# vpc-ccg/haslr

Hardware: AMD Instinct MI355X
Metric: long-read bases/sec through backbone+consensus; GFA match + FASTA %identity (higher is better)
Workload: dtype int32

## Files before the change

### haslr_amd/csrc/kernels/poa.hip

```cpp
#include <type_traits>

#include "kernels.h"

namespace hxk {

namespace {

#include "poa_graph.inl"
#include "poa_dp.inl"
#include "poa_edge.inl"
#include "poa_update.inl"

#define PHASE(k) do { if (tid == 0) { long long _n = clock64(); ph[k] += (unsigned long long)(_n - tc); tc = _n; } } while (0)
#if POA_PHASE_FLAVOUR == POA_PHASE_GUSTAGES
#define GU_T0() do { __syncthreads(); if (tid == 0) tg = clock64(); } while (0)
#define GU_T(k) do { __syncthreads(); if (tid == 0) { long long _n = clock64(); ph[k] += (unsigned long long)(_n - tg); tg = _n; } } while (0)
#else
#define GU_T0() do { } while (0)
#define GU_T(k) do { } while (0)
#endif
#if POA_PHASE_FLAVOUR == POA_PHASE_DPSUB
#define SUBT(k) do { if (tid == 0) { long long _n = clock64(); ph[k] += (unsigned long long)(_n - tc2); tc2 = _n; } } while (0)
#define SUBT0() do { if (tid == 0) tc2 = clock64(); } while (0)
#else
#define SUBT(k) do { } while (0)
#define SUBT0() do { } while (0)
#endif
#define HX_DP_DISPATCH(Lq, Vq, nsq, Tq) do { \
        if (((Lq) + 1 + GM * NP * DL - 1) / (GM * NP * DL) <= (uint32_t)CM) {     \
            dp_rows<CM, DIR, PRUNE, MAXNT == 64>(g, H, Dm, Dw, W, WH, seq, Lq, Vq, ring, R, ring_w, match, mismatch, gap, wmail.box, wmail.consumed, sink_row, sink_score, SINK_LDS, nsq, cl, ph + PW_BUILD0, Tq, (prune_pct >> 16) & 1u, ph + PW_PRUNE0, ED.hrows); \
        } else sOk = ES_INTERNAL; } while (0)

template <int MAXNT, int CM, bool DIR, bool PRUNE>
__device__ __forceinline__ void poa_edge(const uint32_t eidx, const uint32_t mem, const PoaSlot SL, const PoaEdge* __restrict__ edges,
                                         const PoaSeq* __restrict__ seqs, const uint8_t* __restrict__ packed, const uint64_t* __restrict__ read_off,
                                         const uint32_t* __restrict__ read_len, const PoaPools& P, int32_t match, int32_t mismatch, int32_t gap,
                                         char* cns, uint32_t* cns_len, uint32_t* status, unsigned long long* cells, unsigned long long* phase,
                                         uint32_t poll_limit, uint32_t lds_bytes, uint32_t max_indeg, uint32_t dp_lanes, uint32_t prune_pct) {
    __shared__ unsigned long long ph[POA_PHASE_WORDS];
    __shared__ long long tc;
    if (threadIdx.x == 0) { for (int k = 0; k < POA_PHASE_WORDS; k++) ph[k] = 0; tc = clock64(); ph[PW_BEGIN] = pw_pack(pw_lo(wall_clock64(), PW_SPLIT_CLOCK), (unsigned long long)((__builtin_amdgcn_s_getreg(63492) & 0x7fffu) | ((__builtin_amdgcn_s_getreg(63508) & 15u) << 15)), PW_SPLIT_CLOCK); }
#if POA_PHASE_FLAVOUR == POA_PHASE_GUSTAGES
    long long tg = 0;
#endif
#if POA_PHASE_FLAVOUR == POA_PHASE_DPSUB
    __shared__ long long tc2;
#endif
    const PoaEdge ED = edges[eidx];
    const uint32_t tid = threadIdx.x, NT = blockDim.x;
    const uint32_t DL = dp_lanes ? dp_lanes : NT;
    extern __shared__ int32_t ring[];
    G g;
    bind_graph(g, P, SL, ED);
    int32_t* H = P.H + SL.h_off;
    uint8_t* Dm = DIR ? P.dir + SL.d_off : nullptr;
    uint8_t* Dw = DIR ? P.dirw + SL.w_off : nullptr;
    const uint32_t GM = ED.members;
    const uint32_t ring_w = CM * (DL >> 6) * 65u;
    uint32_t R = 0;
    {
        const uint32_t fit = lds_bytes / (ring_w * 4u);
        R = fit >= 8 ? 8 : fit >= 4 ? 4 : fit >= 2 ? 2 : 0;
        if (fit < 1) R = 0xffffffffu;
    }
    uint8_t* seq = P.seq + SL.seq_off;
    const uint32_t W = (ED.lmax + 1 + 31) & ~31u;
    const uint32_t NP = GM == 1 && ED.passes > 1 ? ED.passes : 1u;
    const uint32_t WT = GM * NP * (DL >> 6);
    const uint32_t WH = W + (WT > 1 ? (WT + 3u) & ~3u : 0u);

    constexpr uint32_t SINK_LDS = MAXNT <= 256 ? 128 : MAXNT < 1024 ? 256 : SINK_CAP;
    __shared__ WaveMailT<MAXNT / 64> wmail;
    __shared__ uint32_t lds_u[16];
    __shared__ uint32_t sV, sE, sNaln, sOk, sNsink, sNcand, sBestKey, sWalkN, sWalkI, sWalkJ;
    __shared__ int sBestI;
    __shared__ uint32_t sink_row[SINK_LDS];
    __shared__ int sink_score[SINK_LDS];
    __shared__ uint32_t sCtl;
    __shared__ unsigned long long sCells;
    __shared__ int sPrevScore, sNewT; __shared__ uint32_t sPrevLen, sRetry;
    if (tid == 0) { sV = 0; sE = 0; sOk = R != 0xffffffffu ? ES_OK : ES_INTERNAL; sCells = 0; sPrevScore = 0; sPrevLen = 0; sRetry = 0; sNewT = PRUNE_OFF; }
    if constexpr (MAXNT > 64) {
        for (uint32_t q = tid; q < (MAXNT / 64 - 1) * WAVE_MBOX; q += NT) wmail.box[q] = 0ull;
        if (tid < MAXNT / 64) wmail.consumed[tid] = 0u;
    }
    __syncthreads();
    uint32_t* csy = P.csync + (uint64_t)eidx * CW_STRIDE;
    int32_t* sinkbuf = P.sinkbuf + (uint64_t)eidx * (1 + 2 * SINK_CAP);
    DpCl cl;
    cl.mem = mem; cl.members = GM; cl.stride = ED.vcap + 1; cl.tag0 = 0;
    cl.mbox = P.mbox + (NP > 1 ? SL.mbox_off : ED.cl_off); cl.err = csy + CW_ERR; cl.poll_limit = poll_limit; cl.lanes = DL;
    const uint32_t topo_lcap = lds_bytes >= 24 * 1024 ? 1024u : lds_bytes >= 8 * 1024 ? 256u : 128u;
    const uint32_t topo_lines = lds_bytes >= 24 * 1024 ? 64u : lds_bytes >= 8 * 1024 ? 16u : 8u;
    const uint32_t topo_fixed = topo_lcap * 4 + topo_lines * 256 + topo_lines * 4;
    uint32_t* t_stack = reinterpret_cast<uint32_t*>(ring);
    uint4* t_cache = reinterpret_cast<uint4*>(reinterpret_cast<uint8_t*>(ring) + topo_lcap * 4);
    uint32_t* t_tags = reinterpret_cast<uint32_t*>(reinterpret_cast<uint8_t*>(ring) + topo_lcap * 4 + topo_lines * 256);
    uint8_t* st_lds = reinterpret_cast<uint8_t*>(ring) + topo_fixed;
    uint32_t* tmp_u32 = reinterpret_cast<uint32_t*>(g.pred);
    auto exact_order = [&](uint32_t Vn, uint32_t* out) {
        const bool wave_dfs = topo_fixed + 16 <= lds_bytes;
        const bool st_in_lds = wave_dfs && (uint64_t)Vn + topo_fixed + 16 <= lds_bytes;
        uint8_t* st = st_in_lds ? st_lds : g.mark;
        if (wave_dfs) { for (uint32_t i = tid; i < Vn; i += NT) st[i] = 4u; }
        else { for (uint32_t i = tid; i < Vn; i += NT) { g.mark[i] = 0; g.check[i] = 1; } }
        __threadfence_block();
        __syncthreads();
        if (wave_dfs) {
            uint32_t* ranks = reinterpret_cast<uint32_t*>(g.score);
#if POA_PHASE_FLAVOUR == POA_PHASE_DPSUB
            long long tq0 = clock64();
#endif
            if (tid < 64) toposort_rank(g, Vn, st, t_stack, t_cache, t_tags, ranks, topo_lcap, topo_lines);
#if POA_PHASE_FLAVOUR == POA_PHASE_DPSUB
            if (tid == 0) ph[PW_P2_TOPO] += (unsigned long long)(clock64() - tq0);
#endif
            __threadfence_block();
            __syncthreads();
            for (uint32_t i = tid; i < Vn; i += NT) tmp_u32[i] = g.rank2node[ranks[i]];
            __syncthreads();
            if (out != tmp_u32) { for (uint32_t i = tid; i < Vn; i += NT) out[i] = tmp_u32[i]; }
        } else if (tid == 0) toposort(g, Vn, out);
        __syncthreads();
    };

    uint32_t att = 0;
    for (uint32_t k = ED.seq_begin; mem > 0 || k < ED.seq_end; k += (mem == 0 ? 1u : 0u)) {
        uint32_t L, V;
        if (mem == 0 && sOk != ES_OK) break;
        if (mem == 0) {
            const PoaSeq q = seqs[k];
            L = q.len;
            {
                const uint8_t* rp = packed + read_off[q.rid];
                const uint32_t rlen = read_len[q.rid];
                for (uint32_t j = tid; j < L; j += NT) {
                    uint32_t p = q.strand == 0 ? q.spos + j : rlen - 1 - (q.spos + j);
                    uint8_t b = (rp[p >> 2] >> ((p & 3) * 2)) & 3;
                    seq[j] = q.strand == 0 ? b : (uint8_t)(3 - b);
                }
            }
            __syncthreads();
            PHASE(PW_DECODE);
            V = sV;
            SUBT0();
        } else {
            if (tid == 0) {
                uint32_t v = 0;
                for (uint32_t spin = 0;; spin++) {
                    v = ld_dev(csy + CW_GO);
                    if (v == CL_ABORT || v >= att + 1) break;
                    if (spin > poll_limit) { st_dev(csy + CW_ERR, 1u); v = CL_ABORT; break; }
                    __builtin_amdgcn_s_sleep(32);
                }
                sCtl = v;
            }
            __syncthreads();
            if (sCtl == CL_ABORT) break;
            __builtin_amdgcn_fence(__ATOMIC_ACQUIRE, "agent");
            V = ld_dev(csy + CW_V); L = ld_dev(csy + CW_L);
        }
        if (mem == 0) SUBT(PW_P2_PUBLISH);
        int thrT = PRUNE_OFF;
        if constexpr (PRUNE) {
            if (mem == 0 && (prune_pct & 0xffffu) != 0u && sPrevLen != 0u && V < (1u << 20)) {
                const float f = (float)(prune_pct & 0xffffu) * 0.01f;
                float e = (float)sPrevScore * (float)L / (float)sPrevLen;
                e = e >= 0.f ? e * f : e * (2.f - f);
                thrT = (int)fmaxf((float)PRUNE_OFF, floorf(e));
            }
        }
    redo_dp:
        att++;
        if (GM > 1) {
            if (mem == 0) cluster_publish(csy, V, L, thrT, att);
            else if constexpr (PRUNE) thrT = (int)ld_dev(csy + CW_THRESHOLD);
        }
        if (V > 0) {
            uint32_t ns = 0xffffffffu;
#if POA_PHASE_FLAVOUR == POA_PHASE_MEMBERS
            const long long td0 = clock64();
            if (tid == 0) ph[PW_P3_WAIT] = 0;
#endif
            if (NP > 1) {
                for (uint32_t pass = 0; pass < NP && (uint64_t)pass * DL * CM <= L; pass++) {
                    cl.mem = pass; cl.members = NP;
                    HX_DP_DISPATCH(L, V, ns, thrT);
                    __threadfence();
                    __syncthreads();
                }
                cl.mem = 0; cl.members = 1;
            } else
            HX_DP_DISPATCH(L, V, ns, thrT);
#if POA_PHASE_FLAVOUR == POA_PHASE_MEMBERS
            if (tid == 0 && phase) atomicAdd(&phase[(uint64_t)eidx * POA_PHASE_WORDS + PW_P3_MEMBER0 + min(mem, (uint32_t)(PW_N_BUILD - 1))], pw_pack(0, ph[PW_P3_WAIT] >> 10, PW_SPLIT_HALF) | pw_pack((unsigned long long)(clock64() - td0) >> 10, 0, PW_SPLIT_HALF));
#endif
            if (ns != 0xffffffffu) sNsink = ns;
            cl.tag0 += V;
        }
        if (mem > 0) {
            __syncthreads();
            if (V > 0 && L / (DL * (uint32_t)CM) == mem) {
                const uint32_t nsk = min(sNsink, SINK_LDS);
                if (tid == 0) sinkbuf[0] = (int32_t)sNsink;
                for (uint32_t q = tid; q < nsk; q += NT) { sinkbuf[1 + q] = (int32_t)sink_row[q]; sinkbuf[1 + SINK_CAP + q] = sink_score[q]; }
            }
            __threadfence();
            __syncthreads();
            if (tid == 0) __hip_atomic_fetch_add(csy + CW_DONE, 1u, __ATOMIC_RELAXED, __HIP_MEMORY_SCOPE_AGENT);
            continue;
        }
        SUBT(PW_P2_OWN);
        if (V > 0) {
            if (GM > 1) {
                cluster_wait_members(csy, GM, att, poll_limit);
                __builtin_amdgcn_fence(__ATOMIC_ACQUIRE, "agent");
                if (L / (DL * (uint32_t)CM) != 0) {
                    const uint32_t nsk_all = (uint32_t)sinkbuf[0], nsk = min(nsk_all, SINK_LDS);
                    for (uint32_t q = tid; q < nsk; q += NT) { sink_row[q] = (uint32_t)sinkbuf[1 + q]; sink_score[q] = sinkbuf[1 + SINK_CAP + q]; }
                    if (tid == 0) sNsink = nsk_all;
                }
            }
            __syncthreads();
            if (tid == 0 && ld_dev(csy + CW_ERR) && sOk == ES_OK) sOk = ld_dev(csy + CW_ERR) == 2u ? ES_INTERNAL : ES_STALLED;
            __syncthreads();
            if (sOk != ES_OK) break;
            SUBT(PW_P2_WAIT);
            if (tid == 0) {
                if (sNsink > SINK_LDS) sOk = ES_SINKS;
                int best = INT32_MIN + 1024; uint32_t ncand = 0, first = 0;
                const uint32_t nsk = min(sNsink, SINK_LDS);
                for (uint32_t q = 0; q < nsk; q++) if (sink_score[q] > best) best = sink_score[q];
                for (uint32_t q = 0; q < nsk; q++) if (sink_score[q] == best) { if (!ncand) first = q; sink_row[ncand++] = sink_row[q]; }
                (void)first;
                if constexpr (PRUNE) {
                    sRetry = thrT > PRUNE_OFF && sOk == ES_OK && best < thrT;
                    if (sRetry) { sNewT = nsk ? max(best, PRUNE_OFF) : PRUNE_OFF; ph[PW_PRUNE_REPEATED]++; }
                    else { sPrevScore = best; sPrevLen = L; ph[PW_PRUNE_THRESHOLDS] += thrT > PRUNE_OFF; }
                }
                sNcand = ncand; sBestI = ncand ? (int)sink_row[0] : -1; sBestKey = 0xffffffffu;
                lds_u[WALK_AT_I] = 0; lds_u[WALK_AT_J] = 0; lds_u[WALK_DONE] = 0;
                if (ncand > 1 && ncand <= 8 && lds_bytes >= 640u && !(PRUNE && sRetry)) {
                    constexpr uint32_t UCAP = 32, SCAP = 256;
                    uint32_t* U = reinterpret_cast<uint32_t*>(ring);
                    uint8_t* mk = reinterpret_cast<uint8_t*>(U + UCAP);
                    uint8_t* ck = mk + UCAP;
                    uint8_t* stk = ck + UCAP;
                    uint32_t nu = 0, cn[8];
                    bool ok = true;
                    auto find = [&](uint32_t x) -> uint32_t { for (uint32_t q = 0; q < nu; q++) if (U[q] == x) return q; return NONE; };
                    auto addcol = [&](uint32_t x) {
                        if (find(x) != NONE) return;
                        const uint32_t na = g.n_aligned[x];
                        if (nu + 1 + na > UCAP) { ok = false; return; }
                        U[nu++] = x;
                        for (uint32_t k = 0; k < na; k++) U[nu++] = g.aligned[3 * x + k];
                    };
                    for (uint32_t c = 0; c < ncand; c++) { cn[c] = g.rank2node[sink_row[c] - 1]; if (ok) addcol(cn[c]); }
                    for (uint32_t q = 0; q < nu && ok; q++)
                        for (uint32_t e = g.out_head[U[q]]; e != NONE && ok; e = g.e_next_out[e]) addcol(g.e_to[e]);
                    if (ok) {
                        for (uint32_t q = 1; q < nu; q++) {
                            const uint32_t x = U[q]; uint32_t r = q;
                            while (r > 0 && U[r - 1] > x) { U[r] = U[r - 1]; r--; }
                            U[r] = x;
                        }
                        for (uint32_t q = 0; q < nu; q++) { mk[q] = 0; ck[q] = 1; }
                        auto cand_of = [&](uint32_t x) -> uint32_t { for (uint32_t c = 0; c < ncand; c++) if (cn[c] == x) return c; return NONE; };
                        uint32_t win = NONE;
                        for (uint32_t root = 0; root < nu && win == NONE && ok; root++) {
                            if (mk[root]) continue;
                            uint32_t sp = 0;
                            stk[sp++] = (uint8_t)root;
                            while (sp && win == NONE && ok) {
                                const uint32_t q = stk[sp - 1], n = U[q];
                                bool valid = true;
                                if (mk[q] != 2) {
                                    for (uint32_t e = g.in_head[n]; e != NONE; e = g.e_next_in[e]) {
                                        const uint32_t f = find(g.e_from[e]);
                                        if (f != NONE && mk[f] != 2) { if (sp < SCAP) stk[sp++] = (uint8_t)f; else ok = false; valid = false; }
                                    }
                                    const uint32_t na = g.n_aligned[n];
                                    if (ck[q])
                                        for (uint32_t k = 0; k < na; k++) {
                                            const uint32_t a = find(g.aligned[3 * n + k]);
                                            if (mk[a] != 2) { if (sp < SCAP) stk[sp++] = (uint8_t)a; else ok = false; ck[a] = 0; valid = false; }
                                        }
                                    if (valid) {
                                        mk[q] = 2;
                                        if (ck[q]) {
                                            win = cand_of(n);
                                            for (uint32_t k = 0; k < na && win == NONE; k++) win = cand_of(g.aligned[3 * n + k]);
                                        }
                                    } else mk[q] = 1;
                                }
                                if (valid) sp--;
                            }
                        }
                        if (ok && win != NONE) { sBestI = (int)sink_row[win]; sNcand = 1; }
                    }
                }
            }
            __syncthreads();
            if constexpr (PRUNE) {
                if (sRetry) {
                    thrT = sNewT;
                    __syncthreads();
                    if (tid == 0) sRetry = 0;
                    goto redo_dp;
                }
            }
            if (sNcand > 1 && sOk == ES_OK) {
                if (tid == 0) ph[PW_P2_TIES] += 1;
                exact_order(V, tmp_u32);
                const uint32_t nc = sNcand;
                for (uint32_t r = tid; r < V; r += NT) {
                    const uint32_t n = tmp_u32[r];
                    for (uint32_t q = 0; q < nc; q++)
                        if (g.rank2node[sink_row[q] - 1] == n) atomicMin(&sBestKey, (r << 10) | q);
                }
                __syncthreads();
                if (tid == 0) { sBestI = (int)sink_row[sBestKey & 1023u]; atomicAdd(&ph[PW_ORDER], 0ull); }
            }
            __syncthreads();
            SUBT(PW_P2_END);
            PHASE(PW_DP);
            if (DIR) {
                if (tid < 64) {
                    const uint32_t ln = tid;
                    if (ln == 0) sCells += (unsigned long long)V * L;
                    uint32_t i = (uint32_t)__builtin_amdgcn_readfirstlane(sBestI), j = L, na = 0;
                    int pn = 0, pp = 0;
                    uint32_t nwalk = 0, iend = 0, jend = 0;
                    bool tail = false;
                    while (!(i == 0 && j == 0)) {
                        if (__builtin_expect(na > V + L + 2u, 0)) { if (ln == 0) sOk = ES_INTERNAL; break; }
                        if (i == 0) {
                            if (na & 63u) { const uint32_t base = na & ~63u; if (ln < na - base) { g.aln_node[base + ln] = pn; g.aln_pos[base + ln] = pp; } }
                            tail = true;
                            nwalk = na; iend = 0; jend = j;
                            for (uint32_t q = ln; q < j; q += 64) { g.aln_node[na + q] = -1; g.aln_pos[na + q] = (int32_t)(j - 1 - q); }
                            na += j; j = 0;
                            break;
                        }
                        const uint32_t ti = i, ct = j | 1u;
                        if (NT > 64 && ln == 0) { st_wg(&lds_u[WALK_AT_I], ti); st_wg(&lds_u[WALK_AT_J], ct); }
                        const int32_t bs = ((int32_t)ct - 31) >> 1;
                        uint32_t w0 = 0, w1 = 0, w2 = 0, w3 = 0, mt = 0, pv0 = 0, pv1 = 0, qo = 0, qw = 0;
                        if (ti > ln) {
                            const uint8_t* rowp = Dm + (uint64_t)(ti - ln) * (W >> 1) + bs;
                            __builtin_memcpy(&w0, rowp, 4); __builtin_memcpy(&w1, rowp + 4, 4); __builtin_memcpy(&w2, rowp + 8, 4); __builtin_memcpy(&w3, rowp + 12, 4);
                            const uint32_t rr = ti - 1 - ln;
                            mt = g.row_meta[rr]; qo = g.row_pred_off[rr]; if (mt & 32u) qw = g.wslot[rr];
                            pv0 = (mt >> META_NP) == 0 ? 0u : (g.row_pred0[rr] & 0x0fffffffu) + 1;
                            pv1 = (g.row_pred1[rr] & 0x0fffffffu) + 1;
                        }
                        uint32_t ilo = ti > 63u ? ti - 63u : 1u;
                        asm volatile("" : "+s"(ilo));
                        const int32_t jb0 = 2 * bs;
                        const unsigned long long wmask = __ballot((mt & 32u) != 0);
                        if (mt & 32u) { w0 = 0x88888888u; w1 = 0x88888888u; w2 = 0x88888888u; w3 = 0x88888888u; }
                        for (;;) {
                            const uint32_t dr = ti - i, jb = (uint32_t)((int32_t)j - jb0);
                            const uint32_t wsa = (uint32_t)__builtin_amdgcn_readlane((int)w0, (int)dr), wsb = (uint32_t)__builtin_amdgcn_readlane((int)w1, (int)dr);
                            const uint32_t wsc = (uint32_t)__builtin_amdgcn_readlane((int)w2, (int)dr), wsd = (uint32_t)__builtin_amdgcn_readlane((int)w3, (int)dr);
                            const uint32_t wsh = ((jb & 16u) ? ((jb & 8u) ? wsd : wsc) : ((jb & 8u) ? wsb : wsa)) >> (4 * (jb & 7u));
                            const uint32_t n4 = wsh & 15u;
                            const uint32_t pva = (uint32_t)__builtin_amdgcn_readlane((int)pv0, (int)dr), pvb = (uint32_t)__builtin_amdgcn_readlane((int)pv1, (int)dr);
                            uint32_t ni, nj;
                            asm("s_andn2_b32 %0, 3, %2\n\ts_cselect_b32 %0, %4, %3\n\ts_bitcmp1_b32 %2, 3\n\ts_cselect_b32 %0, %0, %5\n\t"
                                "s_and_b32 %1, %2, 12\n\ts_cmp_lg_u32 %1, 8\n\ts_subb_u32 %1, %6, 0"
                                : "=&s"(ni), "=&s"(nj) : "s"(wsh), "s"(pva), "s"(pvb), "s"(i), "s"(j) : "scc");
                            if (__builtin_expect((n4 & 10u) == 8u, 0)) {
                                uint32_t type = n4 >> 2, slot = 3u - (n4 & 3u), later = 1u, pv = slot == 0 ? pva : pvb;
                                if ((uint32_t)(wmask >> dr) & 1u) {
                                    const uint32_t d = (uint32_t)__builtin_amdgcn_readfirstlane((int)Dw[(uint64_t)__builtin_amdgcn_readlane((int)qw, (int)dr) * W + j]);
                                    type = d >> 4; slot = 15u - (d & 15u); later = slot >= 2 && type > 1u;
                                    pv = slot == 0 ? pva : pvb;
                                }
                                if (later != 0)
                                    pv = ((uint32_t)__builtin_amdgcn_readfirstlane((int)g.pred_rank[(uint32_t)__builtin_amdgcn_readlane((int)qo, (int)dr) + slot]) & 0x0fffffffu) + 1;
                                ni = type > 1u ? pv : i;
                                nj = j - (uint32_t)(type != 2u);
                            }
                            {
                                const int el = (int)(na & 63u);
                                int m0_keep;
                                asm volatile("s_mov_b32 %2, m0\n\ts_mov_b32 m0, %3\n\ts_nop 0\n\tv_writelane_b32 %0, %4, m0\n\tv_writelane_b32 %1, %5, m0\n\ts_mov_b32 m0, %2"
                                             : "+v"(pn), "+v"(pp), "=&s"(m0_keep) : "s"(el), "s"(i), "s"(j));
                            }
                            if (__builtin_expect((na & 63u) == 63u, 0)) {
                                asm volatile("" ::: "memory");
                                g.aln_node[na - 63 + ln] = pn; g.aln_pos[na - 63 + ln] = pp;
                            }
                            na++;
                            i = ni; j = nj;
                            if ((int32_t)((i - ilo) | (uint32_t)((int32_t)j - jb0)) < 0) break;
                        }
                    }
                    if (!tail) {
                        if (na & 63u) { const uint32_t base = na & ~63u; if (ln < na - base) { g.aln_node[base + ln] = pn; g.aln_pos[base + ln] = pp; } }
                        nwalk = na; iend = 0; jend = 0;
                    }
                    if (ln == 0) { sNaln = na; lds_u[WALK_N] = nwalk; lds_u[WALK_I] = iend; lds_u[WALK_J] = jend; st_wg(&lds_u[WALK_DONE], 1u); }
                } else if (tid < 128) {
                    const uint32_t hl = tid - 64u;
                    uint32_t last_i = 0xffffffffu, sink = 0;
                    for (uint32_t spin = 0; spin < (1u << 26); spin++) {
                        if (ld_wg(&lds_u[WALK_DONE])) break;
                        const uint32_t pi_ = ld_wg(&lds_u[WALK_AT_I]), pc = ld_wg(&lds_u[WALK_AT_J]);
                        if (pi_ == last_i) { __builtin_amdgcn_s_sleep(8); continue; }
                        last_i = pi_;
                        for (uint32_t hk = 0; hk < 2; hk++) {
                        const uint32_t d = 64u + hl + 64u * hk;
                        if (pi_ > d) {
                            const uint32_t r = pi_ - d, rr = r - 1;
                            const uint8_t* rowp = Dm + (uint64_t)r * (W >> 1);
                            const uint32_t c_lo = pc > d ? pc - d : 0u, c_hi = pc > d / 3u ? pc - d / 3u : 0u;
                            uint32_t a0, a1;
                            __builtin_memcpy(&a0, rowp + ((c_lo >> 1) & ~3u), 4); __builtin_memcpy(&a1, rowp + ((c_hi >> 1) & ~3u), 4);
                            const uint32_t mt = g.row_meta[rr], qo = g.row_pred_off[rr];
                            sink ^= a0 ^ a1 ^ g.row_pred0[rr] ^ g.row_pred1[rr];
                            if ((mt >> META_NP) > 2u) sink ^= g.pred_rank[qo + 2] ^ g.pred_rank[qo + (mt >> META_NP) - 1];
                            if (mt & 32u) { const uint8_t* wp = Dw + (uint64_t)g.wslot[rr] * W; sink ^= wp[c_lo] ^ wp[(c_lo + c_hi) >> 1] ^ wp[c_hi]; }
                        }
                        }
                    }
                    asm volatile("" :: "v"(sink));
                }
                __syncthreads();
                if (tid == 0) { sWalkN = lds_u[WALK_N]; sWalkI = lds_u[WALK_I]; sWalkJ = lds_u[WALK_J]; }
                __syncthreads();
            } else if (tid == 0) {
                sCells += (unsigned long long)V * L;
                uint32_t i = (uint32_t)sBestI, j = L, na = 0;
                while (!DIR && !(i == 0 && j == 0)) {
                    const int hij = H[(uint64_t)i * WH + j];
                    uint32_t pi_ = i, pj_ = j;
                    bool found = false;
                    uint32_t po = 0, pe = 0;
                    if (i != 0) { po = g.row_pred_off[i - 1]; pe = g.row_pred_off[i]; }
                    if (i != 0 && j != 0) {
                        const int mc = seq[j - 1] == (uint8_t)(g.row_meta[i - 1] & 3u) ? match : mismatch;
                        if (po == pe) { if (hij == H[j - 1] + mc) { pi_ = 0; pj_ = j - 1; found = true; } }
                        else for (uint32_t p = po; p < pe && !found; p++) {
                            uint32_t pr = (g.pred_rank[p] & 0x0fffffffu) + 1;
                            if (hij == H[(uint64_t)pr * WH + j - 1] + mc) { pi_ = pr; pj_ = j - 1; found = true; }
                        }
                    }
                    if (!found && i != 0) {
                        if (po == pe) { if (hij == H[j] + gap) { pi_ = 0; pj_ = j; found = true; } }
                        else for (uint32_t p = po; p < pe && !found; p++) {
                            uint32_t pr = (g.pred_rank[p] & 0x0fffffffu) + 1;
                            if (hij == H[(uint64_t)pr * WH + j] + gap) { pi_ = pr; pj_ = j; found = true; }
                        }
                    }
                    if (!found) { pi_ = i; pj_ = j - 1; }
                    g.aln_node[na] = i == pi_ ? -1 : (int32_t)g.rank2node[i - 1];
                    g.aln_pos[na] = j == pj_ ? -1 : (int32_t)(j - 1);
                    na++;
                    i = pi_; j = pj_;
                }
                sNaln = na; sWalkN = 0;
            }
        } else {
            if (tid == 0) { sNaln = 0; sWalkN = 0; }
            if (GM > 1) cluster_wait_members(csy, GM, att, poll_limit);
        }
        __syncthreads();
        if (sOk != ES_OK) break;
        PHASE(PW_TRACEBACK);
        const uint32_t V_old = sV;
        graph_update(g, seq, L, sNaln, sWalkN, sWalkI, sWalkJ, lds_u, &sV, &sE, &sNcand, &sOk);
        PHASE(PW_GRAPH);
        __syncthreads();
        if (sOk != ES_OK) break;
        order_update(g, V_old, sV, L, lds_u);
        PHASE(PW_ORDER);
        __syncthreads();
        csr_rebuild<MAXNT, DIR>(g, sV, R, max_indeg, ED.hrows, ED.wrows, lds_u, &sOk, ph, phase != nullptr, eidx, k == ED.seq_begin, k + 1 == ED.seq_end);
        __syncthreads();
        PHASE(PW_CSR);
    }
    if (mem > 0) return;
    if (GM > 1 && tid == 0) st_dev(csy + CW_GO, CL_ABORT);
    long long t_cns = 0;
    if (tid == 0) t_cns = clock64();
    if (sOk == ES_OK && sV) {
        if (tid < 64) { const uint32_t cl_ = consensus_fast_wave(g, sV, cns + ED.cns_off); if (tid == 0) sCtl = cl_; }
        __syncthreads();
        if (sCtl == NONE) {
            if (tid == 0) ph[PW_REFCNS] = 1;
            exact_order(sV, g.rank2node);
            for (uint32_t r = tid; r < sV; r += NT) g.node2rank[g.rank2node[r]] = r;
            __syncthreads();
            csr_rebuild<MAXNT, DIR>(g, sV, R, 0xffffffffu, 0xffffffffu, 0xffffffffu, lds_u, &sOk, ph, false, eidx, false, false);
            __threadfence_block();
            __syncthreads();
            if (tid < 64) { const uint32_t cl_ = consensus_wave(g, sV, cns + ED.cns_off); if (tid == 0) sCtl = cl_; }
            __syncthreads();
        }
    }
    if (tid == 0) {
        if (sOk == ES_INTERNAL) { status[eidx] = HXE_SPOS_RANGE << 8; cns_len[eidx] = 0; }
        else if (sOk == ES_OVERFLOW) { status[eidx] = HXE_POA_OVERFLOW; cns_len[eidx] = 0; }
        else if (sOk == ES_NODIR) { status[eidx] = HXE_POA_NODIR; cns_len[eidx] = 0; }
        else if (sOk == ES_FARROWS) { status[eidx] = HXE_POA_FARROWS; cns_len[eidx] = 0; }
        else if (sOk == ES_SINKS) { status[eidx] = HXE_POA_SINKS; cns_len[eidx] = 0; }
        else if (sOk == ES_WIDEROWS) { status[eidx] = HXE_POA_WIDEROWS; cns_len[eidx] = 0; }
        else if (sOk == ES_STALLED) { status[eidx] = HXE_POA_STALLED; cns_len[eidx] = 0; }
        else {
            status[eidx] = 0; cns_len[eidx] = !sV ? 0 : sCtl; atomicAdd(cells, sCells);
#if POA_PHASE_FLAVOUR == POA_PHASE_ROWSTATS
            if (phase) atomicAdd(&ph[PW_SEQS_NODES], pw_pack(0, sV, PW_SPLIT_HALF));
#endif
        }
        ph[PW_CNS] = (unsigned long long)(clock64() - t_cns);
        PHASE(PW_GRAPH);
        ph[PW_END] = pw_lo(wall_clock64(), PW_SPLIT_CLOCK);
#if POA_PHASE_FLAVOUR == POA_PHASE_MEMBERS
        if (phase) for (int k = 0; k < PW_N_PHASES; k++) phase[(uint64_t)eidx * POA_PHASE_WORDS + k] = ph[k];
#else
        if (phase) for (int k = 0; k < POA_PHASE_WORDS; k++) phase[(uint64_t)eidx * POA_PHASE_WORDS + k] = ph[k];
#endif
    }
}
#undef HX_DP_DISPATCH
#undef SUBT0
#undef SUBT
#undef GU_T
#undef GU_T0
#undef PHASE

template <int MAXNT, int CM, bool DIR, bool PERSIST, bool PRUNE>
__global__ void __launch_bounds__(MAXNT, (CM == 8 && DIR ? 4 : 1)) k_poa(const PoaEdge* __restrict__ edges, const uint32_t* __restrict__ order, uint32_t n_items,
                                            const PoaSlot* __restrict__ slots, uint32_t* __restrict__ counter ,
                                            const uint32_t* __restrict__ btab , const PoaSeq* __restrict__ seqs, const uint8_t* __restrict__ packed, const uint64_t* __restrict__ read_off,
                                            const uint32_t* __restrict__ read_len, PoaPools P, int32_t match, int32_t mismatch, int32_t gap,
                                            char* cns, uint32_t* cns_len, uint32_t* status, unsigned long long* cells, unsigned long long* phase,
                                            uint32_t poll_limit, uint32_t lds_bytes, uint32_t max_indeg, uint32_t dp_lanes, uint32_t prune_pct,
                                            uint32_t* __restrict__ started ) {
    __shared__ uint32_t sNext;
    if (started && threadIdx.x == 0) __hip_atomic_fetch_add(started, 1u, __ATOMIC_RELAXED, __HIP_MEMORY_SCOPE_SYSTEM);
    uint32_t kb = 0, nbk = 0;
    bool own_first = false;
    if (PERSIST) { nbk = btab[0] & 0xffffu; own_first = (btab[0] >> 16) & 1u; while (kb + 1 < nbk && blockIdx.x >= btab[1 + kb]) kb++; }
    for (uint32_t round = 0;; round++) {
        uint32_t eidx, mem = 0;
        PoaSlot SL;
        if (!PERSIST) {
            eidx = order[blockIdx.x] & 0x00ffffffu; mem = order[blockIdx.x] >> 24;
            if (eidx == 0x00ffffffu) return;
            SL = slots[edges[eidx].slot];
        } else {
            if (round) __syncthreads();
            if (threadIdx.x == 0) {
                const uint32_t* ib = btab + 1 + nbk;
                const uint32_t* est = ib + nbk + 1;
                uint32_t idx = 0xffffffffu;
                for (uint32_t tries = 0; tries < 64 && idx == 0xffffffffu; tries++) {
                    uint32_t best = 0xffffffffu, bv = 0;
                    for (uint32_t k = kb; k < nbk; k++) {
                        const uint32_t b0 = ib[k], b1 = ib[k + 1], cur = __hip_atomic_load(counter + k, __ATOMIC_RELAXED, __HIP_MEMORY_SCOPE_AGENT);
                        if (cur >= b1 - b0) continue;
                        const uint32_t v = est[b0 + cur];
                        if (best == 0xffffffffu || v > bv) { best = k; bv = v; }
                        if (own_first && k == kb) break;
                    }
                    if (best == 0xffffffffu) break;
                    const uint32_t t = ib[best] + atomicAdd(counter + best, 1u);
                    if (t < ib[best + 1]) idx = t;
                }
                sNext = idx;
            }
            __syncthreads();
            const uint32_t idx = sNext;
            if (idx == 0xffffffffu) return;
            eidx = order[idx] & 0x00ffffffu;
            SL = slots[blockIdx.x];
        }
        poa_edge<MAXNT, CM, DIR, PRUNE>(eidx, mem, SL, edges, seqs, packed, read_off, read_len, P, match, mismatch, gap, cns, cns_len, status, cells, phase, poll_limit, lds_bytes, max_indeg, dp_lanes, prune_pct);
        if (!PERSIST) return;
    }
}

}

#if !defined(HX_POA_PART) || HX_POA_PART == 64
#define HX_POA_HAS_64 1
#endif
#if !defined(HX_POA_PART) || HX_POA_PART == 256
#define HX_POA_HAS_256 1
#endif
#if !defined(HX_POA_PART) || HX_POA_PART == 512
#define HX_POA_HAS_512 1
#endif
#if !defined(HX_POA_PART) || HX_POA_PART == 1024
#define HX_POA_HAS_1024 1
#endif
#define HX_LAUNCH(MNT, CMV, DIRV, PERS, PRN) do { \
        (void)hipFuncSetAttribute((const void*)k_poa<MNT, CMV, DIRV, PERS, PRN>, hipFuncAttributeMaxDynamicSharedMemorySize, 142 * 1024); \
        if (q.occupancy) { (void)hipOccupancyMaxActiveBlocksPerMultiprocessor(q.occupancy, (const void*)k_poa<MNT, CMV, DIRV, PERS, PRN>, q.block_threads, q.ring_bytes); break; } \
        k_poa<MNT, CMV, DIRV, PERS, PRN><<<q.n_blocks, q.block_threads, q.ring_bytes, s>>>(q.edges, q.order, q.n_items, q.slots, q.counter, q.btab, q.seqs, q.packed, q.read_off, q.read_len, q.pools, q.match, q.mismatch, q.gap, \
                                                                       q.cns, q.cns_len, q.status, q.cells, q.phase, q.poll_limit, q.ring_bytes, q.max_indeg, q.dp_lanes, q.prune_pct, q.started); } while (0)
#define HX_LAUNCH_CM(MNT, CMV) do { if (q.use_dir && q.counter) HX_LAUNCH(MNT, CMV, true, true, false); else if (q.use_dir) HX_LAUNCH(MNT, CMV, true, false, false); else HX_LAUNCH(MNT, CMV, false, false, false); } while (0)
#define HX_LAUNCH_PR(MNT, CMV) do { if (q.counter) HX_LAUNCH(MNT, CMV, true, true, true); else HX_LAUNCH(MNT, CMV, true, false, true); } while (0)
#define HX_POA_RUN_PART(MNT, LAST_CM) \
    void poa_run_##MNT(const PoaLaunch& q, hipStream_t s, bool prune) { \
        const int cm = q.cm; \
        if constexpr (MNT == 256 || MNT == 1024) { if (prune && cm <= 2 && !q.counter) { HX_LAUNCH(MNT, 2, true, false, true); return; } } \
        if (prune) { if (cm <= 4) HX_LAUNCH_PR(MNT, 4); else HX_LAUNCH_PR(MNT, 8); return; } \
        if constexpr (MNT == 256 || MNT == 1024) { if (cm <= 2 && q.use_dir && !q.counter) { HX_LAUNCH(MNT, 2, true, false, false); return; } }    \
        if (cm <= 4) HX_LAUNCH_CM(MNT, 4); else if (cm <= 8) HX_LAUNCH_CM(MNT, 8); else if (cm <= 16 || LAST_CM == 16) HX_LAUNCH_CM(MNT, 16); else HX_LAUNCH_CM(MNT, LAST_CM); \
    }
#ifdef HX_POA_HAS_64
HX_POA_RUN_PART(64, 32)
#endif
#ifdef HX_POA_HAS_256
HX_POA_RUN_PART(256, 32)
#endif
#ifdef HX_POA_HAS_512
HX_POA_RUN_PART(512, 16)
#endif
#ifdef HX_POA_HAS_1024
HX_POA_RUN_PART(1024, 32)
#endif
#undef HX_POA_RUN_PART
#undef HX_LAUNCH_CM
#undef HX_LAUNCH_PR
#undef HX_LAUNCH

#if !defined(HX_POA_PART) || HX_POA_PART == 64
void poa_run_64(const PoaLaunch&, hipStream_t, bool);
void poa_run_256(const PoaLaunch&, hipStream_t, bool);
void poa_run_512(const PoaLaunch&, hipStream_t, bool);
void poa_run_1024(const PoaLaunch&, hipStream_t, bool);
void poa_run(const PoaLaunch& q, hipStream_t s) {
    if (!q.n_blocks || !q.n_items) return;
    if (q.counter && !q.use_dir) return;
    const bool prune = poa_prune_ok(q.use_dir, q.cm) && q.prune_pct != 0u;
    const int mnt = poa_kernel_lanes(q.block_threads);
    if (mnt == 64) poa_run_64(q, s, prune);
    else if (mnt == 256) poa_run_256(q, s, prune);
    else if (mnt == 512) poa_run_512(q, s, prune);
    else poa_run_1024(q, s, prune);
}
#endif

}
```

Measured before the change: 2.256 billion.

## Precompute per-lane traceback step table and walk with scalar asm state machine

```diff
diff --git a/haslr_amd/csrc/kernels/poa.hip b/haslr_amd/csrc/kernels/poa.hip
--- a/haslr_amd/csrc/kernels/poa.hip
+++ b/haslr_amd/csrc/kernels/poa.hip
@@ -30,6 +30,33 @@
         if (((Lq) + 1 + GM * NP * DL - 1) / (GM * NP * DL) <= (uint32_t)CM) {     \
             dp_rows<CM, DIR, PRUNE, MAXNT == 64>(g, H, Dm, Dw, W, WH, seq, Lq, Vq, ring, R, ring_w, match, mismatch, gap, wmail.box, wmail.consumed, sink_row, sink_score, SINK_LDS, nsq, cl, ph + PW_BUILD0, Tq, (prune_pct >> 16) & 1u, ph + PW_PRUNE0, ED.hrows); \
         } else sOk = ES_INTERNAL; } while (0)
+
+#define HX_WS(C, T, OFF, RA, RB) \
+    "Ls" #C "_%=:\n\tv_readlane_b32 %[x], %[" T "], %[" RA "]\n\ts_bfe_u32 %[" RB "], %[x], " #OFF "|0x80000\n\ts_cmp_lt_u32 %[" RB "], 64\n\ts_cbranch_scc0 Lx" #C "_%=\n\t" \
+    "s_or_b32 %[w], %[" RA "], (" #C "+2)<<6\n\tv_writelane_b32 %[rec], %[w], m0\n\ts_add_u32 m0, m0, 1\n"
+#define HX_WX(C, RA, RB) \
+    "Lx" #C "_%=:\n\ts_bitcmp1_b32 %[" RB "], 7\n\ts_cbranch_scc1 Ld" #C "_%=\n\ts_cmp_lt_u32 m0, 32\n\ts_cbranch_scc0 Ld" #C "_%=\n\t" \
+    "s_or_b32 %[w], %[" RA "], (" #C "+2)<<6\n\tv_writelane_b32 %[rec], %[w], m0\n\ts_add_u32 m0, m0, 1\n\ts_and_b32 %[" RA "], %[" RB "], 63\n\ts_branch Ls" #C "_%=\n" \
+    "Ld" #C "_%=:\n\ts_mov_b32 %[x], %[" RB "]\n\ts_mov_b32 %[dr], %[" RA "]\n\ts_movk_i32 %[c], " #C "\n\ts_branch Lend_%=\n"
+#define HX_WE(C) "Le" #C "_%=:\n\ts_mov_b32 %[drb], %[dr]\n\ts_branch Ls" #C "_%=\n"
+#define HX_WPAIR(CO, CE, TO, TE, OFF) HX_WS(CO, TO, OFF, "dr", "drb") HX_WS(CE, TE, OFF, "drb", "dr")
+#define HX_WXPAIR(CO, CE) HX_WX(CO, "dr", "drb") HX_WX(CE, "drb", "dr") HX_WE(CE)
+#define HX_WGO(C, L) "s_cmp_eq_u32 %[c], " #C "\n\ts_cbranch_scc1 " L #C "_%=\n\t"
+#define HX_WALK_ASM \
+    "s_mov_b32 %[keep], m0\n\ts_mov_b32 m0, %[el]\n\ts_nop 0\n\t" \
+    "s_cmp_lt_u32 %[c], 8\n\ts_cbranch_scc1 Lg0_%=\n\ts_cmp_lt_u32 %[c], 16\n\ts_cbranch_scc1 Lg1_%=\n\ts_cmp_lt_u32 %[c], 24\n\ts_cbranch_scc1 Lg2_%=\n\t" \
+    HX_WGO(31, "Ls") HX_WGO(30, "Le") HX_WGO(29, "Ls") HX_WGO(28, "Le") HX_WGO(27, "Ls") HX_WGO(26, "Le") HX_WGO(25, "Ls") "s_branch Le24_%=\n" \
+    "Lg2_%=:\n\t" HX_WGO(23, "Ls") HX_WGO(22, "Le") HX_WGO(21, "Ls") HX_WGO(20, "Le") HX_WGO(19, "Ls") HX_WGO(18, "Le") HX_WGO(17, "Ls") "s_branch Le16_%=\n" \
+    "Lg1_%=:\n\t" HX_WGO(15, "Ls") HX_WGO(14, "Le") HX_WGO(13, "Ls") HX_WGO(12, "Le") HX_WGO(11, "Ls") HX_WGO(10, "Le") HX_WGO(9, "Ls") "s_branch Le8_%=\n" \
+    "Lg0_%=:\n\t" HX_WGO(7, "Ls") HX_WGO(6, "Le") HX_WGO(5, "Ls") HX_WGO(4, "Le") HX_WGO(3, "Ls") HX_WGO(2, "Le") HX_WGO(1, "Ls") "s_branch Le0_%=\n" \
+    HX_WPAIR(31, 30, "t7", "t6", 24) HX_WPAIR(29, 28, "t7", "t6", 16) HX_WPAIR(27, 26, "t7", "t6", 8) HX_WPAIR(25, 24, "t7", "t6", 0) \
+    HX_WPAIR(23, 22, "t5", "t4", 24) HX_WPAIR(21, 20, "t5", "t4", 16) HX_WPAIR(19, 18, "t5", "t4", 8) HX_WPAIR(17, 16, "t5", "t4", 0) \
+    HX_WPAIR(15, 14, "t3", "t2", 24) HX_WPAIR(13, 12, "t3", "t2", 16) HX_WPAIR(11, 10, "t3", "t2", 8) HX_WPAIR(9, 8, "t3", "t2", 0) \
+    HX_WPAIR(7, 6, "t1", "t0", 24) HX_WPAIR(5, 4, "t1", "t0", 16) HX_WPAIR(3, 2, "t1", "t0", 8) HX_WPAIR(1, 0, "t1", "t0", 0) \
+    "\ts_mov_b32 %[x], 0\n\ts_branch Lend_%=\n" \
+    HX_WXPAIR(31, 30) HX_WXPAIR(29, 28) HX_WXPAIR(27, 26) HX_WXPAIR(25, 24) HX_WXPAIR(23, 22) HX_WXPAIR(21, 20) HX_WXPAIR(19, 18) HX_WXPAIR(17, 16) \
+    HX_WXPAIR(15, 14) HX_WXPAIR(13, 12) HX_WXPAIR(11, 10) HX_WXPAIR(9, 8) HX_WXPAIR(7, 6) HX_WXPAIR(5, 4) HX_WXPAIR(3, 2) HX_WXPAIR(1, 0) \
+    "Lend_%=:\n\ts_mov_b32 %[el], m0\n\ts_mov_b32 m0, %[keep]"
 
 template <int MAXNT, int CM, bool DIR, bool PRUNE>
 __device__ __forceinline__ void poa_edge(const uint32_t eidx, const uint32_t mem, const PoaSlot SL, const PoaEdge* __restrict__ edges,
@@ -336,7 +363,7 @@
                     while (!(i == 0 && j == 0)) {
                         if (__builtin_expect(na > V + L + 2u, 0)) { if (ln == 0) sOk = ES_INTERNAL; break; }
                         if (i == 0) {
-                            if (na & 63u) { const uint32_t base = na & ~63u; if (ln < na - base) { g.aln_node[base + ln] = pn; g.aln_pos[base + ln] = pp; } }
+                            if constexpr (CM > 4) { if (na & 63u) { const uint32_t base = na & ~63u; if (ln < na - base) { g.aln_node[base + ln] = pn; g.aln_pos[base + ln] = pp; } } }
                             tail = true;
                             nwalk = na; iend = 0; jend = j;
                             for (uint32_t q = ln; q < j; q += 64) { g.aln_node[na + q] = -1; g.aln_pos[na + q] = (int32_t)(j - 1 - q); }
@@ -346,60 +373,144 @@
                         const uint32_t ti = i, ct = j | 1u;
                         if (NT > 64 && ln == 0) { st_wg(&lds_u[WALK_AT_I], ti); st_wg(&lds_u[WALK_AT_J], ct); }
                         const int32_t bs = ((int32_t)ct - 31) >> 1;
-                        uint32_t w0 = 0, w1 = 0, w2 = 0, w3 = 0, mt = 0, pv0 = 0, pv1 = 0, qo = 0, qw = 0;
-                        if (ti > ln) {
-                            const uint8_t* rowp = Dm + (uint64_t)(ti - ln) * (W >> 1) + bs;
-                            __builtin_memcpy(&w0, rowp, 4); __builtin_memcpy(&w1, rowp + 4, 4); __builtin_memcpy(&w2, rowp + 8, 4); __builtin_memcpy(&w3, rowp + 12, 4);
-                            const uint32_t rr = ti - 1 - ln;
-                            mt = g.row_meta[rr]; qo = g.row_pred_off[rr]; if (mt & 32u) qw = g.wslot[rr];
-                            pv0 = (mt >> META_NP) == 0 ? 0u : (g.row_pred0[rr] & 0x0fffffffu) + 1;
-                            pv1 = (g.row_pred1[rr] & 0x0fffffffu) + 1;
-                        }
-                        uint32_t ilo = ti > 63u ? ti - 63u : 1u;
-                        asm volatile("" : "+s"(ilo));
-                        const int32_t jb0 = 2 * bs;
-                        const unsigned long long wmask = __ballot((mt & 32u) != 0);
-                        if (mt & 32u) { w0 = 0x88888888u; w1 = 0x88888888u; w2 = 0x88888888u; w3 = 0x88888888u; }
-                        for (;;) {
-                            const uint32_t dr = ti - i, jb = (uint32_t)((int32_t)j - jb0);
-                            const uint32_t wsa = (uint32_t)__builtin_amdgcn_readlane((int)w0, (int)dr), wsb = (uint32_t)__builtin_amdgcn_readlane((int)w1, (int)dr);
-                            const uint32_t wsc = (uint32_t)__builtin_amdgcn_readlane((int)w2, (int)dr), wsd = (uint32_t)__builtin_amdgcn_readlane((int)w3, (int)dr);
-                            const uint32_t wsh = ((jb & 16u) ? ((jb & 8u) ? wsd : wsc) : ((jb & 8u) ? wsb : wsa)) >> (4 * (jb & 7u));
-                            const uint32_t n4 = wsh & 15u;
-                            const uint32_t pva = (uint32_t)__builtin_amdgcn_readlane((int)pv0, (int)dr), pvb = (uint32_t)__builtin_amdgcn_readlane((int)pv1, (int)dr);
-                            uint32_t ni, nj;
-                            asm("s_andn2_b32 %0, 3, %2\n\ts_cselect_b32 %0, %4, %3\n\ts_bitcmp1_b32 %2, 3\n\ts_cselect_b32 %0, %0, %5\n\t"
-                                "s_and_b32 %1, %2, 12\n\ts_cmp_lg_u32 %1, 8\n\ts_subb_u32 %1, %6, 0"
-                                : "=&s"(ni), "=&s"(nj) : "s"(wsh), "s"(pva), "s"(pvb), "s"(i), "s"(j) : "scc");
-                            if (__builtin_expect((n4 & 10u) == 8u, 0)) {
-                                uint32_t type = n4 >> 2, slot = 3u - (n4 & 3u), later = 1u, pv = slot == 0 ? pva : pvb;
-                                if ((uint32_t)(wmask >> dr) & 1u) {
-                                    const uint32_t d = (uint32_t)__builtin_amdgcn_readfirstlane((int)Dw[(uint64_t)__builtin_amdgcn_readlane((int)qw, (int)dr) * W + j]);
-                                    type = d >> 4; slot = 15u - (d & 15u); later = slot >= 2 && type > 1u;
-                                    pv = slot == 0 ? pva : pvb;
+                        if constexpr (CM <= 4) {
+                            uint32_t w0 = 0, w1 = 0, w2 = 0, w3 = 0, mt = 0, pv0 = 0, pv1 = 0;
+                            if (ti > ln) {
+                                const uint8_t* rowp = Dm + (uint64_t)(ti - ln) * (W >> 1) + bs;
+                                __builtin_memcpy(&w0, rowp, 4); __builtin_memcpy(&w1, rowp + 4, 4); __builtin_memcpy(&w2, rowp + 8, 4); __builtin_memcpy(&w3, rowp + 12, 4);
+                                const uint32_t rr = ti - 1 - ln;
+                                mt = g.row_meta[rr];
+                                pv0 = (mt >> META_NP) == 0 ? 0u : (g.row_pred0[rr] & 0x0fffffffu) + 1;
+                                pv1 = (g.row_pred1[rr] & 0x0fffffffu) + 1;
+                            }
+                            uint32_t ilo = ti > 63u ? ti - 63u : 1u;
+                            asm volatile("" : "+s"(ilo));
+                            const int32_t jb0 = 2 * bs;
+                            const unsigned long long wmask = __ballot((mt & 32u) != 0);
+                            if (mt & 32u) { w0 = 0x88888888u; w1 = 0x88888888u; w2 = 0x88888888u; w3 = 0x88888888u; }
+                            uint32_t tb0, tb1, tb2, tb3, tb4, tb5, tb6, tb7;
+                            {
+                                const bool plain = ti > ln && !(mt & 32u);
+                                const uint32_t t0 = ti - pv0, t1 = ti - pv1;
+                                const uint32_t b0 = plain && pv0 != 0 && t0 > ln && t0 < 64u ? t0 : 0x80u, b1 = plain && pv1 != 0 && t1 > ln && t1 < 64u ? t1 : 0x80u;
+                                const uint32_t lut_lo = 0x40408080u | (b1 << 16) | (b0 << 24), lut_hi = 0x00008080u | (b1 << 16) | (b0 << 24);
+                                const uint32_t hrow = plain ? ln * 0x01010101u : 0x80808080u;
+                                auto cells = [&](uint32_t w, uint32_t& even, uint32_t& odd) {
+                                    const uint32_t x = w ^ 0x88888888u;
+                                    const uint32_t re = __builtin_amdgcn_perm(lut_hi, lut_lo, x & 0x0f0f0f0fu), ro = __builtin_amdgcn_perm(lut_hi, lut_lo, (x >> 4) & 0x0f0f0f0fu);
+                                    even = __builtin_amdgcn_perm(hrow, re, ((x >> 1) & 0x04040404u) | 0x03020100u);
+                                    odd = __builtin_amdgcn_perm(hrow, ro, ((x >> 5) & 0x04040404u) | 0x03020100u);
+                                };
+                                cells(w0, tb0, tb1); cells(w1, tb2, tb3); cells(w2, tb4, tb5); cells(w3, tb6, tb7);
+                            }
+                            uint32_t rec = 0, el = 0, dr = 0, c = (uint32_t)((int32_t)j - jb0);
+                            auto flush = [&]() {
+                                if (ln < el) { g.aln_node[na - el + ln] = (int32_t)(ti - (rec & 63u)); g.aln_pos[na - el + ln] = jb0 + (int32_t)(rec >> 6) - 2; }
+                                el = 0;
+                            };
+                            for (;;) {
+                                if (el >= 32u) flush();
+                                uint32_t x, drb, wrd, m0_keep;
+                                const uint32_t e0 = el;
+                                asm volatile(HX_WALK_ASM
+                                             : [rec] "+v"(rec), [dr] "+s"(dr), [c] "+s"(c), [el] "+s"(el), [x] "=&s"(x), [drb] "=&s"(drb), [w] "=&s"(wrd), [keep] "=&s"(m0_keep)
+                                             : [t0] "v"(tb0), [t1] "v"(tb1), [t2] "v"(tb2), [t3] "v"(tb3), [t4] "v"(tb4), [t5] "v"(tb5), [t6] "v"(tb6), [t7] "v"(tb7)
+                                             : "scc");
+                                na += el - e0;
+                                i = ti - dr;
+                                if (x == 0) { j = (uint32_t)(jb0 - 1); break; }
+                                j = (uint32_t)(jb0 + (int32_t)c);
+                                if (!(x & 0x80u)) continue;
+                                const uint32_t wsa = (uint32_t)__builtin_amdgcn_readlane((int)w0, (int)dr), wsb = (uint32_t)__builtin_amdgcn_readlane((int)w1, (int)dr);
+                                const uint32_t wsc = (uint32_t)__builtin_amdgcn_readlane((int)w2, (int)dr), wsd = (uint32_t)__builtin_amdgcn_readlane((int)w3, (int)dr);
+                                const uint32_t wsh = ((c & 16u) ? ((c & 8u) ? wsd : wsc) : ((c & 8u) ? wsb : wsa)) >> (4 * (c & 7u));
+                                const uint32_t n4 = wsh & 15u;
+                                const uint32_t pva = (uint32_t)__builtin_amdgcn_readlane((int)pv0, (int)dr), pvb = (uint32_t)__builtin_amdgcn_readlane((int)pv1, (int)dr);
+                                uint32_t ni, nj;
+                                asm("s_andn2_b32 %0, 3, %2\n\ts_cselect_b32 %0, %4, %3\n\ts_bitcmp1_b32 %2, 3\n\ts_cselect_b32 %0, %0, %5\n\t"
+                                    "s_and_b32 %1, %2, 12\n\ts_cmp_lg_u32 %1, 8\n\ts_subb_u32 %1, %6, 0"
+                                    : "=&s"(ni), "=&s"(nj) : "s"(wsh), "s"(pva), "s"(pvb), "s"(i), "s"(j) : "scc");
+                                if (__builtin_expect((n4 & 10u) == 8u, 0)) {
+                                    uint32_t type = n4 >> 2, slot = 3u - (n4 & 3u), later = 1u, pv = slot == 0 ? pva : pvb;
+                                    if ((uint32_t)(wmask >> dr) & 1u) {
+                                        const uint32_t d = (uint32_t)__builtin_amdgcn_readfirstlane((int)Dw[(uint64_t)g.wslot[i - 1] * W + j]);
+                                        type = d >> 4; slot = 15u - (d & 15u); later = slot >= 2 && type > 1u;
+                                        pv = slot == 0 ? pva : pvb;
+                                    }
+                                    if (later != 0)
+                                        pv = ((uint32_t)__builtin_amdgcn_readfirstlane((int)g.pred_rank[g.row_pred_off[i - 1] + slot]) & 0x0fffffffu) + 1;
+                                    ni = type > 1u ? pv : i;
+                                    nj = j - (uint32_t)(type != 2u);
                                 }
-                                if (later != 0)
-                                    pv = ((uint32_t)__builtin_amdgcn_readfirstlane((int)g.pred_rank[(uint32_t)__builtin_amdgcn_readlane((int)qo, (int)dr) + slot]) & 0x0fffffffu) + 1;
-                                ni = type > 1u ? pv : i;
-                                nj = j - (uint32_t)(type != 2u);
+                                {
+                                    if (el >= 32u) flush();
+                                    uint32_t keep;
+                                    const uint32_t word = dr | ((c + 2u) << 6);
+                                    asm volatile("s_mov_b32 %1, m0\n\ts_mov_b32 m0, %2\n\ts_nop 0\n\tv_writelane_b32 %0, %3, m0\n\ts_mov_b32 m0, %1"
+                                                 : "+v"(rec), "=&s"(keep) : "s"(el), "s"(word));
+                                    el++; na++;
+                                }
+                                i = ni; j = nj;
+                                if ((int32_t)((i - ilo) | (uint32_t)((int32_t)j - jb0)) < 0) break;
+                                dr = ti - i; c = (uint32_t)((int32_t)j - jb0);
                             }
-                            {
-                                const int el = (int)(na & 63u);
-                                int m0_keep;
-                                asm volatile("s_mov_b32 %2, m0\n\ts_mov_b32 m0, %3\n\ts_nop 0\n\tv_writelane_b32 %0, %4, m0\n\tv_writelane_b32 %1, %5, m0\n\ts_mov_b32 m0, %2"
-                                             : "+v"(pn), "+v"(pp), "=&s"(m0_keep) : "s"(el), "s"(i), "s"(j));
+                            flush();
+                        } else {
+                            uint32_t w0 = 0, w1 = 0, w2 = 0, w3 = 0, mt = 0, pv0 = 0, pv1 = 0, qo = 0, qw = 0;
+                            if (ti > ln) {
+                                const uint8_t* rowp = Dm + (uint64_t)(ti - ln) * (W >> 1) + bs;
+                                __builtin_memcpy(&w0, rowp, 4); __builtin_memcpy(&w1, rowp + 4, 4); __builtin_memcpy(&w2, rowp + 8, 4); __builtin_memcpy(&w3, rowp + 12, 4);
+                                const uint32_t rr = ti - 1 - ln;
+                                mt = g.row_meta[rr]; qo = g.row_pred_off[rr]; if (mt & 32u) qw = g.wslot[rr];
+                                pv0 = (mt >> META_NP) == 0 ? 0u : (g.row_pred0[rr] & 0x0fffffffu) + 1;
+                                pv1 = (g.row_pred1[rr] & 0x0fffffffu) + 1;
                             }
-                            if (__builtin_expect((na & 63u) == 63u, 0)) {
-                                asm volatile("" ::: "memory");
-                                g.aln_node[na - 63 + ln] = pn; g.aln_pos[na - 63 + ln] = pp;
+                            uint32_t ilo = ti > 63u ? ti - 63u : 1u;
+                            asm volatile("" : "+s"(ilo));
+                            const int32_t jb0 = 2 * bs;
+                            const unsigned long long wmask = __ballot((mt & 32u) != 0);
+                            if (mt & 32u) { w0 = 0x88888888u; w1 = 0x88888888u; w2 = 0x88888888u; w3 = 0x88888888u; }
+                            for (;;) {
+                                const uint32_t dr = ti - i, jb = (uint32_t)((int32_t)j - jb0);
+                                const uint32_t wsa = (uint32_t)__builtin_amdgcn_readlane((int)w0, (int)dr), wsb = (uint32_t)__builtin_amdgcn_readlane((int)w1, (int)dr);
+                                const uint32_t wsc = (uint32_t)__builtin_amdgcn_readlane((int)w2, (int)dr), wsd = (uint32_t)__builtin_amdgcn_readlane((int)w3, (int)dr);
+                                const uint32_t wsh = ((jb & 16u) ? ((jb & 8u) ? wsd : wsc) : ((jb & 8u) ? wsb : wsa)) >> (4 * (jb & 7u));
+                                const uint32_t n4 = wsh & 15u;
+                                const uint32_t pva = (uint32_t)__builtin_amdgcn_readlane((int)pv0, (int)dr), pvb = (uint32_t)__builtin_amdgcn_readlane((int)pv1, (int)dr);
+                                uint32_t ni, nj;
+                                asm("s_andn2_b32 %0, 3, %2\n\ts_cselect_b32 %0, %4, %3\n\ts_bitcmp1_b32 %2, 3\n\ts_cselect_b32 %0, %0, %5\n\t"
+                                    "s_and_b32 %1, %2, 12\n\ts_cmp_lg_u32 %1, 8\n\ts_subb_u32 %1, %6, 0"
+                                    : "=&s"(ni), "=&s"(nj) : "s"(wsh), "s"(pva), "s"(pvb), "s"(i), "s"(j) : "scc");
+                                if (__builtin_expect((n4 & 10u) == 8u, 0)) {
+                                    uint32_t type = n4 >> 2, slot = 3u - (n4 & 3u), later = 1u, pv = slot == 0 ? pva : pvb;
+                                    if ((uint32_t)(wmask >> dr) & 1u) {
+                                        const uint32_t d = (uint32_t)__builtin_amdgcn_readfirstlane((int)Dw[(uint64_t)__builtin_amdgcn_readlane((int)qw, (int)dr) * W + j]);
+                                        type = d >> 4; slot = 15u - (d & 15u); later = slot >= 2 && type > 1u;
+                                        pv = slot == 0 ? pva : pvb;
+                                    }
+                                    if (later != 0)
+                                        pv = ((uint32_t)__builtin_amdgcn_readfirstlane((int)g.pred_rank[(uint32_t)__builtin_amdgcn_readlane((int)qo, (int)dr) + slot]) & 0x0fffffffu) + 1;
+                                    ni = type > 1u ? pv : i;
+                                    nj = j - (uint32_t)(type != 2u);
+                                }
+                                {
+                                    const int el = (int)(na & 63u);
+                                    int m0_keep;
+                                    asm volatile("s_mov_b32 %2, m0\n\ts_mov_b32 m0, %3\n\ts_nop 0\n\tv_writelane_b32 %0, %4, m0\n\tv_writelane_b32 %1, %5, m0\n\ts_mov_b32 m0, %2"
+                                                 : "+v"(pn), "+v"(pp), "=&s"(m0_keep) : "s"(el), "s"(i), "s"(j));
+                                }
+                                if (__builtin_expect((na & 63u) == 63u, 0)) {
+                                    asm volatile("" ::: "memory");
+                                    g.aln_node[na - 63 + ln] = pn; g.aln_pos[na - 63 + ln] = pp;
+                                }
+                                na++;
+                                i = ni; j = nj;
+                                if ((int32_t)((i - ilo) | (uint32_t)((int32_t)j - jb0)) < 0) break;
                             }
-                            na++;
-                            i = ni; j = nj;
-                            if ((int32_t)((i - ilo) | (uint32_t)((int32_t)j - jb0)) < 0) break;
                         }
                     }
                     if (!tail) {
-                        if (na & 63u) { const uint32_t base = na & ~63u; if (ln < na - base) { g.aln_node[base + ln] = pn; g.aln_pos[base + ln] = pp; } }
+                        if constexpr (CM > 4) { if (na & 63u) { const uint32_t base = na & ~63u; if (ln < na - base) { g.aln_node[base + ln] = pn; g.aln_pos[base + ln] = pp; } } }
                         nwalk = na; iend = 0; jend = 0;
                     }
                     if (ln == 0) { sNaln = na; lds_u[WALK_N] = nwalk; lds_u[WALK_I] = iend; lds_u[WALK_J] = jend; st_wg(&lds_u[WALK_DONE], 1u); }
```

Result: faster. 2.360 billion, median of 6 (+4.6%).
